# jiny2001/dcscn-super-resolution

Hardware: NVIDIA H100
Metric: output Mpixels/sec DCSCN L12 x2 (higher is better)
Workload: dtype f16x3 (fp16 hi/lo split operands, fp32 accumulate; fp32-equivalent)

## Files before the change

### dcscn-super-resolution_b200/csrc/conv_tc.cuh

```cuda
#pragma once
#include "common.h"
#include "epilogue.cuh"
#include "ptx.cuh"

namespace dcscn {

constexpr int kConsumerWGs = 2;
constexpr int kTcThreads = (1 + kConsumerWGs) * 128;
constexpr int kRegsIssue = 40, kRegsEpilogue = 232;
constexpr int kMaxASlots = 4;
constexpr int kMaxWSlots = 12;
constexpr int kTcBarrierBytes = 2 * (kMaxASlots + kMaxWSlots) * 8;
constexpr int kMaxTileN = 112;
constexpr int kRdotSmemBytes = 9 * 128 * 4;
constexpr int kColSplit = 2;
constexpr int kXchgStride = 36;
constexpr int kXchgBytes = kConsumerWGs * 64 * kXchgStride * 4;
constexpr int kTcKC = 64;

struct TcSmem {
  static constexpr int kRowBytes = kTcKC * 2;
  static constexpr int kSbo = 8 * kRowBytes;
  static constexpr uint64_t kLayout = 1ull;
};

__device__ __forceinline__ uint64_t make_smem_desc(uint32_t saddr) {
  return (uint64_t)((saddr & 0x3FFFFu) >> 4) | ((uint64_t)1 << 16) | ((uint64_t)(TcSmem::kSbo >> 4) << 32) |
         (TcSmem::kLayout << 62);
}

__host__ __device__ inline uint32_t tc_a_plane_bytes(int TW, int TH, int ksz) {
  return ((uint32_t)TW * (uint32_t)(TH + ksz - 1) * (uint32_t)kTcKC * 2u + 1023u) & ~1023u;
}
__host__ __device__ inline uint32_t tc_w_tile_bytes(int nplanes, int n_pad) {
  return (uint32_t)nplanes * (uint32_t)n_pad * (uint32_t)kTcKC * 2u;
}

template <int N, int NPLANES, int KS>
__device__ __forceinline__ void tile_products(float (&corr)[N / 2], float (&dom)[N / 2], uint64_t a_hi, uint64_t a_lo,
                                              uint64_t b_hi, uint64_t b_lo, uint32_t acc_on) {
  ptx::wgmma_fence();
#pragma unroll
  for (int ks = 0; ks < KS; ++ks) {
    const uint64_t kadd = (uint64_t)ks * 2u;
    const uint32_t on = ks == 0 ? acc_on : 1u;
    if (NPLANES == 2) {
      ptx::wgmma_f16<N, 0, 0>(corr, a_lo + kadd, b_hi + kadd, on);
      ptx::wgmma_f16<N, 0, 0>(corr, a_hi + kadd, b_lo + kadd, 1u);
    }
    ptx::wgmma_f16<N, 0, 0>(dom, a_hi + kadd, b_hi + kadd, on);
  }
  ptx::wgmma_commit();
}

template <int NPLANES, int N>
__global__ void __launch_bounds__(kTcThreads, 1)
conv_tc_kernel(const __grid_constant__ CUtensorMap tm_hi, const __grid_constant__ CUtensorMap tm_lo,
               const ConvTCParams p, const int a_slots, const int w_slots) {
  static_assert(N % 16 == 0 && N >= 16 && N <= kMaxTileN, "column tile width");
  extern __shared__ __align__(1024) uint8_t smem_raw[];
  uint8_t* smem = reinterpret_cast<uint8_t*>((reinterpret_cast<uintptr_t>(smem_raw) + 1023) & ~uintptr_t(1023));
  const ConvGeom& g = p.g;
  const int ksz = p.ksz;
  const uint32_t A_PLANE = tc_a_plane_bytes(g.TW, g.TH, ksz);
  const uint32_t A_SLOT = NPLANES * A_PLANE;
  const uint32_t A_TX = (uint32_t)NPLANES * (uint32_t)g.TW * (uint32_t)(g.TH + ksz - 1) * kTcKC * 2u;
  constexpr uint32_t B_BYTES = N * kTcKC * 2;
  constexpr uint32_t W_TILE = NPLANES * B_BYTES;
  uint8_t* a_ring = smem;
  uint8_t* w_ring = smem + (size_t)a_slots * A_SLOT;
  uint64_t* a_full = reinterpret_cast<uint64_t*>(w_ring + (size_t)w_slots * W_TILE);
  uint64_t* a_empty = a_full + kMaxASlots;
  uint64_t* w_full = a_empty + kMaxASlots;
  uint64_t* w_empty = w_full + kMaxWSlots;
  float* s_rdot = reinterpret_cast<float*>(w_empty + kMaxWSlots);
  float* s_xchg = s_rdot + kRdotSmemBytes / 4;

  const int wg = threadIdx.x >> 7;
  const int lane = threadIdx.x & 31;

  if (threadIdx.x == 0) {
    for (int s = 0; s < a_slots; ++s) {
      ptx::mbar_init(&a_full[s], 1);
      ptx::mbar_init(&a_empty[s], kConsumerWGs);
    }
    for (int s = 0; s < w_slots; ++s) {
      ptx::mbar_init(&w_full[s], 1);
      ptx::mbar_init(&w_empty[s], kConsumerWGs);
    }
    ptx::fence_barrier_init();
    ptx::fence_proxy_async();
  }
  if (p.epi.mode == EPI_D2S_RDOT)
    for (int i = threadIdx.x; i < p.epi.rdot_taps * p.epi.d2s_cout; i += blockDim.x) s_rdot[i] = p.epi.rdot_w[i];
  __syncthreads();

  const int tiles_per_img = g.tiles_x * g.tiles_y;
  const int num_items = g.n_img * tiles_per_img * p.n_tiles;
  const int half = ksz >> 1;
  const int chunks = p.chunks;

  if (wg == 0) {
    ptx::setmaxnreg_dec<kRegsIssue>();
    if (threadIdx.x == 0) {
      ptx::prefetch_tensormap(&tm_hi);
      if (NPLANES == 2) ptx::prefetch_tensormap(&tm_lo);
      int as = 0, ws = 0;
      uint32_t a_ph = 0, w_ph = 0;
      for (int item = blockIdx.x; item < num_items; item += gridDim.x) {
        const int n_tile = item % p.n_tiles;
        const int tile = item / p.n_tiles;
        const int img = tile / tiles_per_img;
        const int t2 = tile - img * tiles_per_img;
        const int ty = t2 / g.tiles_x, tx = t2 - ty * g.tiles_x;
        const int x0 = tx * g.TW - half, y0 = ty * g.TH - half;
        const uint8_t* wsrc = reinterpret_cast<const uint8_t*>(p.wpack) + (size_t)n_tile * ksz * ksz * chunks * W_TILE;
        for (int ch = 0; ch < chunks; ++ch) {
          for (int dx = 0; dx < ksz; ++dx) {
            ptx::mbar_wait(&a_empty[as], a_ph ^ 1);
            uint8_t* ad = a_ring + (size_t)as * A_SLOT;
            ptx::mbar_arrive_expect_tx(&a_full[as], A_TX);
            ptx::tma_load_4d(ad, &tm_hi, &a_full[as], ch * kTcKC, x0 + dx, y0, img);
            if (NPLANES == 2) ptx::tma_load_4d(ad + A_PLANE, &tm_lo, &a_full[as], ch * kTcKC, x0 + dx, y0, img);
            if (++as == a_slots) { as = 0; a_ph ^= 1; }
            for (int dy = 0; dy < ksz; ++dy) {
              ptx::mbar_wait(&w_empty[ws], w_ph ^ 1);
              uint8_t* wd = w_ring + (size_t)ws * W_TILE;
              ptx::mbar_arrive_expect_tx(&w_full[ws], W_TILE);
              const uint8_t* wtile = wsrc + (size_t)((dy * ksz + dx) * chunks + ch) * W_TILE;
              ptx::bulk_load(wd, wtile, W_TILE, &w_full[ws]);
              if (++ws == w_slots) { ws = 0; w_ph ^= 1; }
            }
          }
        }
      }
    }
  } else {
    ptx::setmaxnreg_inc<kRegsEpilogue>();
    const int cw = wg - 1;
    const int t = threadIdx.x & 127;
    const int wq = t >> 5;
    constexpr int nch = N >> 4;
    constexpr int per = (nch + kColSplit - 1) / kColSplit;
    const int n_total = p.n_tiles * N;
    const bool strict = p.seg_chunks == 1;
    const uint32_t a_ring_u32 = ptx::smem_u32(a_ring);
    const uint32_t w_ring_u32 = ptx::smem_u32(w_ring);
    const uint32_t a_off = (uint32_t)(cw * 64 * TcSmem::kRowBytes);
    const uint32_t dy_step = (uint32_t)(g.TW * TcSmem::kRowBytes);
    const int row = cw * 64 + (t >> 1);
    const int grp = t & 1;
    const int py = row / g.TW, px = row - py * g.TW;
    const int first_chunk = grp * per;
    const int my_chunks = (nch - first_chunk) < per ? ((nch - first_chunk) > 0 ? nch - first_chunk : 0) : per;
    float* xchg = s_xchg + cw * 64 * kXchgStride;
    auto release_a = [&](int s) { ptx::mbar_arrive_if(&a_empty[s], t == 0); };
    auto release_w = [&](int s) { ptx::mbar_arrive_if(&w_empty[s], t == 0); };
    int as = 0, ws = 0;
    uint32_t a_ph = 0, w_ph = 0;
    for (int item = blockIdx.x; item < num_items; item += gridDim.x) {
      const int n_tile = item % p.n_tiles;
      const int tile = item / p.n_tiles;
      const int img = tile / tiles_per_img;
      const int t2 = tile - img * tiles_per_img;
      const int ty = t2 / g.tiles_x, tx = t2 - ty * g.tiles_x;
      const int y = ty * g.TH + py, x = tx * g.TW + px;
      const bool valid = (y < g.H) && (x < g.W);

      float sum[N / 2], corr[N / 2], dom[N / 2];
#pragma unroll
      for (int i = 0; i < N / 2; ++i) sum[i] = 0.f;
      auto promote = [&]() {
        ptx::reg_fence(corr);
        ptx::reg_fence(dom);
#pragma unroll
        for (int i = 0; i < N / 2; ++i) {
          if (NPLANES == 2) sum[i] += corr[i];
          sum[i] += dom[i];
        }
      };
      uint32_t acc_on = 0;
      int seg_left = p.seg_chunks;
      int pend_w = -1, pend_a = -1;
      for (int ch = 0; ch < chunks; ++ch) {
        int ksteps = p.cin_pad - ch * kTcKC;
        ksteps = (ksteps > kTcKC ? kTcKC : ksteps) >> 4;
        for (int dx = 0; dx < ksz; ++dx) {
          ptx::mbar_wait(&a_full[as], a_ph);
          const uint32_t a_addr = a_ring_u32 + (uint32_t)as * A_SLOT + a_off;
          for (int dy = 0; dy < ksz; ++dy) {
            ptx::mbar_wait(&w_full[ws], w_ph);
            const uint32_t w_addr = w_ring_u32 + (uint32_t)ws * W_TILE;
            const uint64_t a_hi = make_smem_desc(a_addr + (uint32_t)dy * dy_step);
            const uint64_t a_lo = make_smem_desc(a_addr + (uint32_t)dy * dy_step + A_PLANE);
            const uint64_t b_hi = make_smem_desc(w_addr);
            const uint64_t b_lo = make_smem_desc(w_addr + B_BYTES);
            const bool a_done = dy == ksz - 1;
            if (strict) {
#pragma unroll 1
              for (int ks = 0; ks < ksteps; ++ks) {
                const uint64_t kadd = (uint64_t)ks * 2u;
                tile_products<N, NPLANES, 1>(corr, dom, a_hi + kadd, a_lo + kadd, b_hi + kadd, b_lo + kadd, acc_on);
                ptx::wgmma_wait<0>();
                promote();
              }
              release_w(ws);
              if (a_done) release_a(as);
            } else {
              if (ksteps == 4)
                tile_products<N, NPLANES, 4>(corr, dom, a_hi, a_lo, b_hi, b_lo, acc_on);
              else if (ksteps == 1)
                tile_products<N, NPLANES, 1>(corr, dom, a_hi, a_lo, b_hi, b_lo, acc_on);
              else if (ksteps == 2)
                tile_products<N, NPLANES, 2>(corr, dom, a_hi, a_lo, b_hi, b_lo, acc_on);
              else
                tile_products<N, NPLANES, 3>(corr, dom, a_hi, a_lo, b_hi, b_lo, acc_on);
              acc_on = 1;
              const bool item_end = a_done && dx == ksz - 1 && ch == chunks - 1;
              if (--seg_left == 0 || item_end) {
                ptx::wgmma_wait<0>();
                promote();
                acc_on = 0;
                seg_left = p.seg_chunks;
                if (pend_w >= 0) release_w(pend_w);
                if (pend_a >= 0) release_a(pend_a);
                release_w(ws);
                if (a_done) release_a(as);
                pend_w = pend_a = -1;
              } else {
                ptx::wgmma_wait<1>();
                if (pend_w >= 0) release_w(pend_w);
                if (pend_a >= 0) release_a(pend_a);
                pend_w = ws;
                pend_a = a_done ? as : -1;
              }
            }
            if (++ws == w_slots) { ws = 0; w_ph ^= 1; }
          }
          if (++as == a_slots) { as = 0; a_ph ^= 1; }
        }
      }
      ptx::wgmma_wait<0>();

      float v9[9];
#pragma unroll
      for (int i = 0; i < 9; ++i) v9[i] = 0.f;
      const int r0 = wq * 16 + (lane >> 2), cq = 2 * (lane & 3);
#pragma unroll
      for (int k = 0; k < per; ++k) {
        ptx::named_bar_sync(1 + cw, 128);
#pragma unroll
        for (int c = 0; c < nch; ++c) {
          if (c == k || c == per + k) {
            float* dst = xchg + (c == k ? 0 : 16);
#pragma unroll
            for (int h = 0; h < 2; ++h) {
              const int j = 2 * c + h;
              dst[r0 * kXchgStride + 8 * h + cq] = sum[4 * j];
              dst[r0 * kXchgStride + 8 * h + cq + 1] = sum[4 * j + 1];
              dst[(r0 + 8) * kXchgStride + 8 * h + cq] = sum[4 * j + 2];
              dst[(r0 + 8) * kXchgStride + 8 * h + cq + 1] = sum[4 * j + 3];
            }
          }
        }
        ptx::named_bar_sync(1 + cw, 128);
        if (k < my_chunks) {
          float v[16];
          const float4* srcp = reinterpret_cast<const float4*>(xchg + (t >> 1) * kXchgStride + grp * 16);
#pragma unroll
          for (int q = 0; q < 4; ++q) {
            const float4 f = srcp[q];
            v[4 * q] = f.x; v[4 * q + 1] = f.y; v[4 * q + 2] = f.z; v[4 * q + 3] = f.w;
          }
          const int cg = n_tile * N + (first_chunk + k) * 16;
          if (p.epi.mode == EPI_D2S_RDOT) {
            if (cg < p.epi.n_valid) {
              const int ij = cg / p.epi.d2s_cout, cc = cg - ij * p.epi.d2s_cout;
              rdot_accumulate16(p.epi, s_rdot, cg, cc, v, v9);
              const bool last = p.epi.rdot_parts > 1 ? k + 1 == my_chunks : cc + 16 == p.epi.d2s_cout;
              if (last && valid) rdot_flush(p.epi, g, img, y, x, ij, p.epi.rdot_parts > 1 ? cc / (per * 16) : 0, v9);
            }
          } else if (valid) {
            if (p.epi.mode == EPI_D2S_TAPS) taps_store16(p.epi, g, img, y, x, cg, v);
            else epilogue_store16(p.epi, g, n_total, img, y, x, cg, v);
          }
        }
      }
    }
  }

  __syncthreads();
}

}
```

### dcscn-super-resolution_b200/csrc/engine.cu

```cuda
#include <cuda.h>
#include <cudaTypedefs.h>
#include <cuda_fp16.h>
#include <cuda_runtime.h>

#include <algorithm>
#include <cmath>
#include <cstdarg>
#include <cstdio>
#include <cstring>
#include <map>
#include <memory>
#include <string>
#include <type_traits>
#include <utility>
#include <vector>

#include "../../include/dcscn_b200.h"
#include "common.h"
#include "conv_aux.cuh"
#include "conv_tc.cuh"
#include "conv_ds_tile.cuh"
#include "train.cuh"
#include "wgrad_tc.cuh"
#include "train_ds.cuh"
// ... 636 lines not shown
      if (rdot_fusable(np, fuse_unit)) {
        t.n_pad = np;
        t.n_tiles = (cout_cols + np - 1) / np;
        break;
      }
    }
  }
  t.n_valid = cout_cols;
  t.w_host.assign((size_t)ksz * ksz * cin * cout_cols, 0.f);
  t.bias_host.assign((size_t)t.n_tiles * t.n_pad, 0.f);
  t.alpha_host.assign((size_t)t.n_tiles * t.n_pad, 1.f);
  return t;
}

static int finalize_params_ds(dcscn_handle* h) {
  h->ds_ab = dcscn_handle::DsDev();
  h->ds.clear();
  h->ds.resize(h->layers.size());
  const int T = h->ds_total, L = h->cfg.layers;
  std::vector<float> ab_pw, ab_bias, ab_alpha;
  const int na = h->cfg.nin_filters, nb = h->cfg.nin_filters2;
  ab_pw.assign((size_t)T * (na + nb), 0.f);
  ab_bias.assign(na + nb, 0.f);
  ab_alpha.assign(na + nb, 1.f);
  const bool slopes = h->cfg.activator <= DCSCN_ACTIVATOR_LEAKY_RELU;
  for (size_t i = 0; i < h->layers.size(); ++i) {
    const LayerDef& l = h->layers[i];
    const std::vector<float>& dwv = P(h, l.scope + "/depthwise_W");
    const std::vector<float>& pwv = P(h, l.scope + "/pointwise_W");
    if (l.scope == "A1" || l.scope == "B1") {
      const int col0 = l.scope == "A1" ? 0 : na;
      int ci = 0;
      for (int li = 0; li < L; ++li)
        for (int k = 0; k < h->filters[li]; ++k, ++ci) {
          const int pos = h->ds_off[li] + k;
          for (int co = 0; co < l.cout; ++co)
            if (l.k == 1) ab_pw[(size_t)pos * (na + nb) + col0 + co] = dwv[ci] * pwv[(size_t)ci * l.cout + co];
        }
      const auto& B = P(h, l.scope + "/conv_B");
      for (int co = 0; co < l.cout; ++co) ab_bias[col0 + co] = B[co];
      layer_slopes(h, l, ab_alpha.data() + col0);
      continue;
    }
    if (h->ds[i].dw.upload(dwv) || h->ds[i].pw.upload(pwv)) return 1;
    if (l.bias && h->ds[i].bias.upload(P(h, l.scope + "/conv_B"))) return 1;
    if (l.act) {
      std::vector<float> a(l.cout);
      layer_slopes(h, l, a.data());
      if (slopes && h->ds[i].alpha.upload(a)) return 1;
    }
  }
  if (h->ds_ab.pw.upload(ab_pw) || h->ds_ab.bias.upload(ab_bias)) return 1;
  if (slopes && h->ds_ab.alpha.upload(ab_alpha)) return 1;
  h->params_dirty = false;
  return 0;
}

static int build_bwd_layers(dcscn_handle* h);
static int sync_host_params(dcscn_handle* h);

static void first_layer_vectors(const dcscn_handle* h, std::vector<float>& w, std::vector<float>& b, std::vector<float>& a) {
  const LayerDef* l = find_layer(h, "CNN1");
  const int taps = l->k * l->k, np = h->feat_w[0];
  w.assign((size_t)taps * np, 0.f);
  b.assign(np, 0.f);
  a.assign(np, 1.f);
  std::vector<float> tmp;
  const std::vector<float>& W = layer_filter(h, *l, tmp);
  for (int tp = 0; tp < taps; ++tp)
    for (int co = 0; co < l->cout; ++co) w[(size_t)tp * np + co] = W[(size_t)tp * l->cout + co];
  const auto& B = P(h, "CNN1/conv_B");
  for (int co = 0; co < l->cout; ++co) b[co] = B[co];
  layer_slopes(h, *l, a.data());
}

static int construct_tc_layers(dcscn_handle* h) {
  const dcscn_config& c = h->cfg;
  const int L = c.layers;
  for (int i = 1; i < L; ++i) {
    const std::string scope = "CNN" + std::to_string(i + 1);
    const LayerDef* l = find_layer(h, scope);
    TcLayer t = make_tc(scope, tc_ksz(h, *l), l->cin, l->cout, h->feat_w[i - 1]);
    for (int ci = 0; ci < l->cin; ++ci) t.in_map.push_back(ci);
    fuse_columns(h, t, scope, 0, 0);
    h->tcl.push_back(std::move(t));
  }
  {
    const LayerDef* a1 = find_layer(h, "A1");
    const LayerDef* b1 = find_layer(h, "B1");
    TcLayer t = make_tc("A1+B1", 1, a1->cin, h->a1_w + b1->cout, h->feat_pitch);
    for (int li = 0; li < L; ++li)
      for (int ci = 0; ci < h->filters[li]; ++ci) t.in_map.push_back(h->feat_off[li] + ci);
    fuse_columns(h, t, "A1", 0, 0);
    fuse_columns(h, t, "B1", h->a1_w, 0);
    h->tcl.push_back(std::move(t));
  }
  {
    const LayerDef* l = find_layer(h, "B2");
    TcLayer t = make_tc("B2", tc_ksz(h, *l), l->cin, l->cout, h->b1_w);
    for (int ci = 0; ci < l->cin; ++ci) t.in_map.push_back(ci);
    fuse_columns(h, t, "B2", 0, 0);
    h->tcl.push_back(std::move(t));
  }
  {
    const std::string scope = up_scope(h);
    const LayerDef* l = find_layer(h, scope);
    const int fuse_unit = find_layer(h, "R-CNN1")->k == 3 ? h->ps_out : 0;
    TcLayer t = make_tc(tconv(h) ? "Up-TCNN" : "Up-PS", tc_ksz(h, *l), l->cin, l->cout, h->nin_pitch,
                        two_stage_up(h) ? 0 : fuse_unit);
    for (int ci = 0; ci < c.nin_filters2; ++ci) t.in_map.push_back(ci);
    for (int ci = 0; ci < c.nin_filters; ++ci) t.in_map.push_back(h->b1_w + ci);
    fuse_columns(h, t, scope, 0, 0);
    h->tcl.push_back(std::move(t));
    if (two_stage_up(h)) {
      const LayerDef* l2 = find_layer(h, "Up-PS2/Up-PS2_CNN");
      TcLayer t2 = make_tc("Up-PS2", tc_ksz(h, *l2), l2->cin, l2->cout, h->mid_pitch, fuse_unit);
      for (int ci = 0; ci < l2->cin; ++ci) t2.in_map.push_back(ci);
      fuse_columns(h, t2, "Up-PS2/Up-PS2_CNN", 0, 0);
      h->tcl.push_back(std::move(t2));
    }
  }
  if (h->train_enabled && !uses_ds_tile(h) && build_bwd_layers(h)) return 1;
  return 0;
}

static int rdot_parts(int n_pad, int cout) {
  const int nch = n_pad >> 4, per16 = ((nch + kColSplit - 1) / kColSplit) * 16;
  if (cout <= 0 || per16 % cout == 0) return 1;
  return (cout % per16 == 0) ? cout / per16 : 1;
}

static bool last_fuses(const dcscn_handle* h, int n_pad) {
  const int cout = h->ps_out, nch = n_pad >> 4, per = (nch + kColSplit - 1) / kColSplit;
  return find_layer(h, "R-CNN1")->k == 3 && cout % 16 == 0 && cout <= 128 && nch % kColSplit == 0 &&
         ((per * 16) % cout == 0 || (rdot_parts(n_pad, cout) > 1 && n_pad % (per * 16) == 0));
}

static double fold_dot(const float* a, const float* w, int C) {
  double s = 0.0;
  for (int c = 0; c < C; ++c) s += (double)a[c] * (double)w[c];
  return s;
}

static TcLayer fold_shape(const TcLayer& up, int C) {
  TcLayer f;
  f.name = up.name;
  f.ksz = up.ksz;
  f.cin = up.cin;
  f.cin_pad = up.cin_pad;
  f.in_map = up.in_map;
  f.cout = f.n_valid = up.cout / C * 9;
  f.n_pad = up.n_pad;
  f.n_tiles = (f.cout + f.n_pad - 1) / f.n_pad;
  f.w_host.assign((size_t)f.ksz * f.ksz * f.cin * f.cout, 0.f);
  f.bias_host.assign((size_t)f.n_tiles * f.n_pad, 0.f);
  f.alpha_host.assign((size_t)f.n_tiles * f.n_pad, 1.f);
  f.dw_ksz = up.dw_ksz;
  f.dw_host = up.dw_host;
  return f;
}

static void build_fold(dcscn_handle* h) {
  h->fold = TcLayer();
  const TcLayer& up = h->tcl.back();
  if (planes(h) != 2 || !last_fuses(h, up.n_pad)) return;
  std::vector<float> tmp;
  const std::vector<float>& wr = layer_filter(h, *find_layer(h, "R-CNN1"), tmp);
  const int C = h->ps_out, sub = up.cout / C;
  TcLayer f = fold_shape(up, C);
  const size_t rows = (size_t)up.ksz * up.ksz * up.cin;
  for (size_t r = 0; r < rows; ++r)
    for (int ij = 0; ij < sub; ++ij)
      for (int t = 0; t < 9; ++t)
        f.w_host[r * f.cout + ij * 9 + t] = (float)fold_dot(&up.w_host[r * up.cout + (size_t)ij * C], &wr[(size_t)t * C], C);
  for (int ij = 0; ij < sub; ++ij)
    for (int t = 0; t < 9; ++t) f.bias_host[ij * 9 + t] = (float)fold_dot(&up.bias_host[(size_t)ij * C], &wr[(size_t)t * C], C);
  h->fold = std::move(f);
}

static void adopt_arrays(TcLayer& t, TcLayer& old) {
  t.d_wpack = std::move(old.d_wpack); t.d_bias = std::move(old.d_bias); t.d_alpha = std::move(old.d_alpha);
  t.d_wref = std::move(old.d_wref); t.d_in_map = std::move(old.d_in_map); t.d_img_map = std::move(old.d_img_map);
  t.d_dw = std::move(old.d_dw);
}

static int finalize_params(dcscn_handle* h) {
  const dcscn_config& c = h->cfg;
  if (sync_host_params(h)) return 1;
  if (uses_ds_tile(h)) return finalize_params_ds(h);
  std::vector<TcLayer> old_tcl = std::move(h->tcl);
  std::vector<TcLayer> old_bwd = std::move(h->bwd);
  TcLayer old_fold = std::move(h->fold);
  h->tcl.clear();
  h->bwd.clear();
  h->refresh_ready = false;
  bool moved = false;
  {
    std::vector<float> w, b, a;
    first_layer_vectors(h, w, b, a);
    if (h->d_first_w.upload(w, &moved) || h->d_first_bias.upload(b, &moved) || h->d_first_alpha.upload(a, &moved)) return 1;
  }
  if (construct_tc_layers(h)) return 1;
  auto repack = [&](std::vector<TcLayer>& cur, std::vector<TcLayer>& old) {
    for (size_t i = 0; i < cur.size(); ++i) {
      TcLayer& t = cur[i];
      if (i < old.size()) adopt_arrays(t, old[i]);
      if (pack_tc_layer(h, t, &moved)) return 1;
    }
    return 0;
  };
  if (repack(h->tcl, old_tcl) || repack(h->bwd, old_bwd)) return 1;
  build_fold(h);
  if (h->fold.cout > 0) {
    adopt_arrays(h->fold, old_fold);
    if (pack_tc_layer(h, h->fold, &moved)) return 1;
  }
  {
    std::vector<float> tmp;
    if (h->d_last_w.upload(layer_filter(h, *find_layer(h, "R-CNN1"), tmp), &moved)) return 1;
  }
  if (moved) {
    h->plans.clear();
    h->last_plan = nullptr;
  }
  h->graph_epoch++;
  h->params_dirty = false;
  return 0;
}

struct WorkspaceShape {
  size_t feat, b1, nin, mid;
  size_t u;
  size_t hr, vbuf;
  int planes;
  size_t bytes_per_px(bool ds) const {
    return ds ? 4 * (feat + b1 + nin + mid + hr) : 2 * (size_t)planes * (feat + b1 + nin + mid + u) + 4 * (hr + vbuf);
  }
};

static WorkspaceShape workspace_shape(const dcscn_handle* h) {
  const dcscn_config& c = h->cfg;
  const size_t s2 = (size_t)c.scale * c.scale;
  WorkspaceShape w;
  w.u = 0;
  if (uses_ds_tile(h)) {
    const int cps = c.nin_filters + c.nin_filters2;
    w.feat = h->ds_total;
    w.b1 = c.nin_filters2;
    w.nin = cps;
    w.mid = c.scale == 4 ? 4 * (size_t)cps : 0;
    w.hr = s2 * h->ps_out;
    w.vbuf = 0;
    w.planes = 1;
    return w;
  }
  w.feat = h->feat_pitch;
  w.b1 = h->b1_w;
  w.nin = h->nin_pitch;
  w.mid = two_stage_up(h) ? 4 * (size_t)h->mid_pitch : 0;
  w.hr = s2 * h->ps_out;
  w.vbuf = s2 * 9 * (size_t)rdot_parts(h->tcl.empty() ? 16 : h->tcl.back().n_pad, h->ps_out);
  w.planes = planes(h);
  if (h->ds_wide) {
    for (const LayerDef& l : h->layers) {
      if (!ds_split(h, l)) continue;
      const std::string& sc = l.scope;
      const size_t per_px = sc == "B2" ? w.b1 : sc == "Up-PS/Up-PS_CNN" ? w.nin : sc == "Up-PS2/Up-PS2_CNN" ? w.mid
                                                                          : (size_t)pad16(l.cin);
      w.u = std::max(w.u, per_px);
    }
  }
  return w;
}

static int ensure_workspace(dcscn_handle* h, size_t lr_px) {
  if (lr_px <= h->cap_px) return 0;
  const dcscn_config& c = h->cfg;
  const WorkspaceShape ws = workspace_shape(h);
  if (uses_ds_tile(h)) {
    if (h->ds_feat.alloc(lr_px * ws.feat, true)) return 1;
    if (h->ds_b1.alloc(lr_px * ws.b1) || h->ds_nin.alloc(lr_px * ws.nin)) return 1;
    if (c.scale == 4 && h->ds_mid.alloc(lr_px * ws.mid)) return 1;
    if (h->ds_hr.alloc(lr_px * ws.hr)) return 1;
    h->cap_px = lr_px;
    return 0;
  }
  h->plans.clear();
  h->last_plan = nullptr;
  const bool two = ws.planes == 2;
  if (h->feat.alloc(lr_px * ws.feat, two) || h->b1.alloc(lr_px * ws.b1, two) || h->nin.alloc(lr_px * ws.nin, two) ||
      h->mid.alloc(lr_px * ws.mid, two) || h->u.alloc(lr_px * ws.u, two))
    return 1;
  if (h->hr.alloc(lr_px * ws.hr, true) || h->vbuf.alloc(lr_px * ws.vbuf, true)) return 1;
  h->cap_px = lr_px;
  return 0;
}

static int64_t workspace_bytes(const dcscn_handle* h) {
  auto bytes = [](const auto&... a) { return (int64_t)(0 + ... + (a.size() * sizeof(*a.get()))); };
  return h->feat.bytes() + h->b1.bytes() + h->nin.bytes() + h->mid.bytes() + h->u.bytes() +
         bytes(h->hr, h->vbuf, h->ds_feat, h->ds_b1, h->ds_nin, h->ds_mid, h->ds_hr, h->tile_x, h->tile_x2, h->tile_y);
}

constexpr size_t kTcRingBudget = 227 * 1024 - 1024 - kTcBarrierBytes - kRdotSmemBytes - kXchgBytes;

static bool tc_patch_fits(int nplanes, int n_pad, int ksz, int TH, int TW) {
  if (ksz == 1) return true;
  if (TW % 8 != 0) return false;
  return 2 * (size_t)nplanes * tc_a_plane_bytes(TW, TH, ksz) + 2 * (size_t)tc_w_tile_bytes(nplanes, n_pad) <=
         kTcRingBudget;
}

static bool choose_patch(int H, int W, int nplanes, int n_pad, int ksz, int* TH, int* TW) {
  static const int cand[][2] = {{8, 16}, {4, 32}, {16, 8}, {2, 64}, {32, 4}, {1, 128}, {64, 2}, {128, 1}};
  long long best = -1;
  for (auto& c : cand) {
    const int th = c[0], tw = c[1];
    if (!tc_patch_fits(nplanes, n_pad, ksz, th, tw)) continue;
    long long area = (long long)((H + th - 1) / th) * th * ((W + tw - 1) / tw) * tw;
    if (best < 0 || area < best) {
      best = area;
      *TH = th;
      *TW = tw;
    }
  }
  return best >= 0;
}

static int encode_map(dcscn_handle* h, CUtensorMap* tm, const __half* base, int cin_pad, int pitch, int n, int H,
                      int W, int TH, int TW) {
  cuuint64_t dims[4] = {(cuuint64_t)cin_pad, (cuuint64_t)W, (cuuint64_t)H, (cuuint64_t)n};
  cuuint64_t strides[3] = {(cuuint64_t)pitch * 2, (cuuint64_t)W * pitch * 2, (cuuint64_t)H * W * pitch * 2};
  cuuint32_t box[4] = {(cuuint32_t)kTcKC, (cuuint32_t)TW, (cuuint32_t)TH, 1};
  cuuint32_t estr[4] = {1, 1, 1, 1};
  CUresult r = h->encode(tm, CU_TENSOR_MAP_DATA_TYPE_FLOAT16, 4, (void*)base, dims, strides, box, estr,
                         CU_TENSOR_MAP_INTERLEAVE_NONE, CU_TENSOR_MAP_SWIZZLE_128B,
                         CU_TENSOR_MAP_L2_PROMOTION_L2_256B, CU_TENSOR_MAP_FLOAT_OOB_FILL_NONE);
  if (r != CUDA_SUCCESS)
    return fail("cuTensorMapEncodeTiled failed (%d) cin_pad=%d pitch=%d n=%d H=%d W=%d box=%dx%d", (int)r, cin_pad,
                pitch, n, H, W, TH, TW);
  return 0;
}

static int add_tc_launch(dcscn_handle* h, Plan* pl, const TcLayer& t, PlaneView src, int src_pitch, int n, int H, int W,
                         const EpiParams& epi) {
  TcLaunch L;
  memset(&L, 0, sizeof(L));
  int TH = 0, TW = 0;
  if (!choose_patch(H, W, planes(h), t.n_pad, t.ksz, &TH, &TW))
    return fail("layer %s: no pixel patch fits a %dx%d filter in shared memory", t.name.c_str(), t.ksz, t.ksz);
  if (t.ksz > 1 && TW % 8 != 0)
    return fail("internal: layer %s: patch width %d is not a whole number of swizzle atoms", t.name.c_str(), TW);
  ConvGeom g{n, H, W, (W + TW - 1) / TW, (H + TH - 1) / TH, TW, TH};
  const int box_rows = TH + t.ksz - 1;
  if (encode_map(h, &L.tm_hi, src.hi, t.cin_pad, src_pitch, n, H, W, box_rows, TW)) return 1;
  if (planes(h) == 2) {
    if (encode_map(h, &L.tm_lo, src.lo, t.cin_pad, src_pitch, n, H, W, box_rows, TW)) return 1;
  } else {
    L.tm_lo = L.tm_hi;
  }
  L.p.g = g;
  L.p.ksz = t.ksz;
  L.p.cin_pad = t.cin_pad;
  L.p.chunks = (t.cin_pad + kTcKC - 1) / kTcKC;
  L.p.n_tiles = t.n_tiles;
  L.p.n_pad = t.n_pad;
  L.p.seg_chunks = h->seg_chunks > 0 ? h->seg_chunks : (t.n_pad > 64 ? 2 : 3);
  L.p.wpack = t.d_wpack.get();
  L.p.epi = epi;
  L.p.epi.bias = t.d_bias.get();
  L.p.epi.alpha = t.d_alpha.get();
  L.p.epi.out_scale = 1.0f / t.wscale;
  if (!h->tcl.empty() && &t >= h->tcl.data() && &t < h->tcl.data() + h->tcl.size()) {
    L.layer_index = (int)(&t - h->tcl.data());
    L.layer_bwd = false;
  } else if (!h->bwd.empty() && &t >= h->bwd.data() && &t < h->bwd.data() + h->bwd.size()) {
    L.layer_index = (int)(&t - h->bwd.data());
    L.layer_bwd = true;
  }
  L.p.epi.n_valid = t.n_valid;

  const size_t a_slot = (size_t)planes(h) * tc_a_plane_bytes(TW, TH, t.ksz);
  const size_t w_tile = tc_w_tile_bytes(planes(h), t.n_pad);
  const size_t budget = kTcRingBudget;
  int a_slots, w_slots;
  if (t.ksz == 1) {
    a_slots = w_slots = (int)std::min<size_t>(kMaxASlots, budget / (a_slot + w_tile));
  } else {
    a_slots = 3;
    if (budget < a_slots * a_slot + 4 * w_tile) a_slots = 2;
    w_slots = budget < a_slots * a_slot ? 0 : (int)std::min<size_t>(kMaxWSlots, (budget - a_slots * a_slot) / w_tile);
  }
  if (a_slots < 2 || w_slots < 2)
    return fail("layer %s: two %zu-byte activation slots and two %zu-byte weight tiles do not fit in shared memory",
                t.name.c_str(), a_slot, w_tile);
  L.a_slots = a_slots;
  L.w_slots = w_slots;
  L.smem = a_slots * a_slot + w_slots * w_tile + 1024 + kTcBarrierBytes + kRdotSmemBytes + kXchgBytes;
  const long long tiles = (long long)n * g.tiles_x * g.tiles_y;
  const long long items = tiles * t.n_tiles;
  L.grid = (int)std::min<long long>(items, h->sm_count);

  L.ref.g = g;
  L.ref.ksz = t.ksz;
  L.ref.cin = t.cin;
  L.ref.cout = t.cout;
  L.ref.src_hi = src.hi;
  L.ref.src_lo = src.lo;
  L.ref.src_pitch = src_pitch;
  L.ref.in_map = t.d_in_map.get();
  L.ref.w = t.d_wref.get();
  L.ref.n_total_pad = t.n_tiles * t.n_pad;
  L.ref.epi = L.p.epi;
  L.ref.epi.out_scale = 1.0f;
  pl->tc.push_back(L);
  return 0;
}

static int add_layer_launch(dcscn_handle* h, Plan* pl, const TcLayer& t, PlaneView src, int src_pitch, int n, int H, int W,
                            const EpiParams& epi) {
  DwParams d;
  memset(&d, 0, sizeof(d));
  if (t.dw_ksz) {
    const PlaneView u = h->u.at(0);
    d = DwParams{n, H, W, t.dw_ksz, t.cin_pad, src.hi, src.lo, src_pitch, t.d_dw.get(), u.hi, u.lo};
    src = u;
    src_pitch = t.cin_pad;
    pl->dw_count++;
  }
  pl->dw.push_back(d);
  return add_tc_launch(h, pl, t, src, src_pitch, n, H, W, epi);
}

static EpiParams epi_planes(PlaneView dst, int pitch, int cols) {
  EpiParams e;
  memset(&e, 0, sizeof(e));
  e.mode = EPI_PLANES;
  e.num_seg = 1;
  e.seg[0] = {0, cols, dst.hi, dst.lo, pitch};
  e.keep_prob = 1.0f;
  e.out_scale = 1.0f;
  return e;
}

static EpiParams epi_activated(const dcscn_handle* h, std::initializer_list<const ActView*> outs) {
  EpiParams e = epi_planes({}, 0, 0);
  e.num_seg = 0;
  for (const ActView* v : outs) {
    e.seg[e.num_seg++] = {v->drop_col0, v->drop_col0 + pad16(v->ch), v->planes.hi, v->planes.lo, v->pitch};
    e.drop_ntotal = v->drop_stride;
  }
  e.act = h->cfg.activator;
  return e;
}

static int add_activated_launch(dcscn_handle* h, Plan* pl, const TcLayer& t, const ActView& src, int n, int H, int W,
                                std::initializer_list<const ActView*> outs) {
  if (add_layer_launch(h, pl, t, src.planes, src.pitch, n, H, W, epi_activated(h, outs))) return 1;
  std::copy(outs.begin(), outs.end(), pl->tc.back().act);
  return 0;
}

static Plan* get_plan(dcscn_handle* h, int n, int H, int W) {
  for (auto& p : h->plans)
    if (p->n == n && p->h == H && p->w == W) return p.get();
  const dcscn_config& c = h->cfg;
  const int L = c.layers;
  std::unique_ptr<Plan> pl(new Plan());
  pl->n = n;
  pl->h = H;
  pl->w = W;
  pl->act.resize(h->layers.size());
  for (size_t li = 0; li < h->layers.size(); ++li)
    if (h->layers[li].act) act_view(h, h->layers[li].scope, &pl->act[li]);
  const ActView* a = pl->act.data();

  memset(&pl->first, 0, sizeof(pl->first));
  pl->first.g = ConvGeom{n, H, W, 1, 1, 1, 1};
  pl->first.ksz = find_layer(h, "CNN1")->k;
  pl->first.n_pad = h->feat_w[0];
  pl->first.w = h->d_first_w.get();
  pl->first.epi = epi_activated(h, {&a[0]});
  pl->first.epi.bias = h->d_first_bias.get();
  pl->first.epi.alpha = h->d_first_alpha.get();
  pl->first.epi.n_valid = h->filters[0];

  size_t ti = 0;
  for (int i = 1; i < L; ++i)
    if (add_activated_launch(h, pl.get(), h->tcl[ti++], a[i - 1], n, H, W, {&a[i]})) return nullptr;
  if (add_activated_launch(h, pl.get(), h->tcl[ti++], a[0], n, H, W, {&a[L], &a[L + 1]})) return nullptr;
  if (add_activated_launch(h, pl.get(), h->tcl[ti++], a[L + 1], n, H, W, {&a[L + 2]})) return nullptr;
  int HR_H = H, HR_W = W;
  {
    EpiParams e;
    memset(&e, 0, sizeof(e));
    e.keep_prob = 1.0f;
    if (two_stage_up(h)) {
      e.mode = EPI_D2S_PLANES;
      e.d2s_r = 2;
      e.d2s_cout = c.nin_filters + c.nin_filters2;
      e.num_seg = 1;
      e.seg[0] = {0, 0, h->mid.hi.get(), h->mid.lo.get(), h->mid_pitch};
    } else {
      e.mode = EPI_D2S_F32;
      e.d2s_r = c.scale;
      e.d2s_cout = h->ps_out;
      e.dst_f32 = h->hr.get();
      e.d2s_pitch = h->ps_out;
    }
    if (add_layer_launch(h, pl.get(), h->tcl[ti++], h->nin.at(0), h->nin_pitch, n, H, W, e)) return nullptr;
    HR_H = H * (two_stage_up(h) ? 2 : c.scale);
    HR_W = W * (two_stage_up(h) ? 2 : c.scale);
  }
  if (two_stage_up(h)) {
    EpiParams e;
    memset(&e, 0, sizeof(e));
    e.keep_prob = 1.0f;
    e.mode = EPI_D2S_F32;
    e.d2s_r = 2;
    e.d2s_cout = h->ps_out;
    e.dst_f32 = h->hr.get();
    e.d2s_pitch = h->ps_out;
    if (add_layer_launch(h, pl.get(), h->tcl[ti++], h->mid.at(0), h->mid_pitch, n, HR_H, HR_W, e)) return nullptr;
    HR_H *= 2;
    HR_W *= 2;
  }
  {
    TcLaunch& L = pl->tc.back();
    const int cout = h->ps_out, nch = L.p.n_pad >> 4, per = (nch + kColSplit - 1) / kColSplit;
    const int klast = find_layer(h, "R-CNN1")->k;
    const int parts = rdot_parts(L.p.n_pad, cout);
    pl->unfused = L;
    pl->fused_index = (int)pl->tc.size() - 1;
    pl->fused_last = last_fuses(h, L.p.n_pad);
    if (pl->fused_last && h->fold.cout > 0) {
      const TcLayer& f = h->fold;
      L.layer_index = -1;
      L.layer_fold = true;
      L.p.n_tiles = f.n_tiles;
      L.p.wpack = f.d_wpack.get();
      L.p.epi.bias = f.d_bias.get();
      L.p.epi.alpha = f.d_alpha.get();
      L.p.epi.out_scale = 1.0f / f.wscale;
      L.p.epi.n_valid = f.n_valid;
      L.p.epi.mode = EPI_D2S_TAPS;
      L.p.epi.rdot_out = h->vbuf.get();
      L.p.epi.rdot_taps = 9;
      L.p.epi.rdot_parts = 1;
      L.grid = (int)std::min<long long>((long long)n * L.p.g.tiles_x * L.p.g.tiles_y * f.n_tiles, h->sm_count);
    } else if (pl->fused_last) {
      L.p.epi.rdot_parts = ((per * 16) % cout == 0) ? 1 : parts;
      L.p.epi.mode = EPI_D2S_RDOT;
      L.p.epi.rdot_w = h->d_last_w.get();
      L.p.epi.rdot_out = h->vbuf.get();
      L.p.epi.rdot_taps = klast * klast;
    }
    const int gparts = pl->fused_last ? L.p.epi.rdot_parts : 1;
    memset(&pl->gather, 0, sizeof(pl->gather));
    pl->gather.parts = gparts;
    pl->gather.n_img = n;
    pl->gather.H = HR_H;
    pl->gather.W = HR_W;
    pl->gather.ksz = klast;
    pl->gather.v = h->vbuf.get();
  }
  memset(&pl->last, 0, sizeof(pl->last));
  pl->last.n_img = n;
  pl->last.H = HR_H;
  pl->last.W = HR_W;
  pl->last.ksz = find_layer(h, "R-CNN1")->k;
  pl->last.C = h->ps_out;
  pl->last.pitch = h->ps_out;
  pl->last.src = h->hr.get();
  pl->last.w = h->d_last_w.get();
  pl->last.bias = 0.f;
  if (h->plans.size() >= 64) h->plans.erase(h->plans.begin());
  h->plans.push_back(std::move(pl));
  return h->plans.back().get();
}

template <int NPL, int N>
static int launch_tc_inst(dcscn_handle* h, const TcLaunch& L, cudaStream_t st) {
  static bool attr_set_dev[64] = {};
  bool& attr_set = attr_set_dev[h->cfg.device_id & 63];
  if (!attr_set) {
    CUDA_TRY(cudaFuncSetAttribute(conv_tc_kernel<NPL, N>, cudaFuncAttributeMaxDynamicSharedMemorySize, 227 * 1024));
    attr_set = true;
  }
  conv_tc_kernel<NPL, N><<<L.grid, kTcThreads, L.smem, st>>>(L.tm_hi, L.tm_lo, L.p, L.a_slots, L.w_slots);
  CUDA_TRY(cudaGetLastError());
  return 0;
}

template <int NPL>
static int launch_tc_width(dcscn_handle* h, const TcLaunch& L, cudaStream_t st) {
  switch (L.p.n_pad) {
    case 16: return launch_tc_inst<NPL, 16>(h, L, st);
    case 32: return launch_tc_inst<NPL, 32>(h, L, st);
    case 48: return launch_tc_inst<NPL, 48>(h, L, st);
    case 64: return launch_tc_inst<NPL, 64>(h, L, st);
    case 80: return launch_tc_inst<NPL, 80>(h, L, st);
    case 96: return launch_tc_inst<NPL, 96>(h, L, st);
    case 112: return launch_tc_inst<NPL, 112>(h, L, st);
  }
  return fail("internal: column tile width %d is not a multiple of 16 in [16, %d]", L.p.n_pad, kMaxTileN);
}

static int launch_tc(dcscn_handle* h, const TcLaunch& Lc, cudaStream_t st) {
  h->launches++;
  TcLaunch& L = const_cast<TcLaunch&>(Lc);
  if (L.layer_fold) {
    L.p.epi.out_scale = 1.0f / h->fold.wscale;
  } else if (L.layer_index >= 0) {
    const std::vector<TcLayer>& ls = L.layer_bwd ? h->bwd : h->tcl;
    if (L.layer_index < (int)ls.size()) L.p.epi.out_scale = 1.0f / ls[L.layer_index].wscale;
  }
  if (h->conv_impl == 1) {
    const long long total = (long long)L.ref.g.n_img * L.ref.g.H * L.ref.g.W * (L.ref.n_total_pad >> 4);
    const int grid = (int)std::min<long long>((total + 127) / 128, (long long)h->sm_count * 16);
    conv_ref_kernel<<<grid, 128, 0, st>>>(L.ref);
    CUDA_TRY(cudaGetLastError());
    return 0;
  }
  const int npl = planes(h);
  if (L.p.wpack == nullptr) return fail("internal: weight image was not packed for this layer");
  return npl == 2 ? launch_tc_width<2>(h, L, st) : launch_tc_width<1>(h, L, st);
}

static int mark(dcscn_handle* h, cudaStream_t st) {
  if (!h->timing) return 0;
  if (h->ev_used >= (int)h->ev.size()) {
    cudaEvent_t e;
    CUDA_TRY(cudaEventCreate(&e));
    h->ev.emplace_back(e);
  }
  CUDA_TRY(cudaEventRecord(h->ev[h->ev_used++].get(), st));
  return 0;
}

template <int KSZ>
static int launch_ds_tile_k(dcscn_handle* h, const DsTileParams& p, unsigned grid, size_t smem, cudaStream_t st) {
  const int cols = p.cout < 32 ? ((p.cout + 3) & ~3) : 32;
  static size_t attr_dev[64][2] = {};
  size_t& cur = attr_dev[h->cfg.device_id & 63][KSZ == 3 ? 1 : 0];
  if (cur == 0) cur = 48 * 1024;
  if (smem > cur) {
    const int b = (int)smem;
    CUDA_TRY(cudaFuncSetAttribute(ds_tile_kernel<KSZ, 1>, cudaFuncAttributeMaxDynamicSharedMemorySize, b));
    CUDA_TRY(cudaFuncSetAttribute(ds_tile_kernel<KSZ, 2>, cudaFuncAttributeMaxDynamicSharedMemorySize, b));
    CUDA_TRY(cudaFuncSetAttribute(ds_tile_kernel<KSZ, 4>, cudaFuncAttributeMaxDynamicSharedMemorySize, b));
    CUDA_TRY(cudaFuncSetAttribute(ds_tile_kernel<KSZ, 6>, cudaFuncAttributeMaxDynamicSharedMemorySize, b));
    CUDA_TRY(cudaFuncSetAttribute(ds_tile_kernel<KSZ, 8>, cudaFuncAttributeMaxDynamicSharedMemorySize, b));
    cur = smem;
  }
  if (cols <= 4) ds_tile_kernel<KSZ, 1><<<grid, kDtThreads, smem, st>>>(p);
  else if (cols <= 8) ds_tile_kernel<KSZ, 2><<<grid, kDtThreads, smem, st>>>(p);
  else if (cols <= 16) ds_tile_kernel<KSZ, 4><<<grid, kDtThreads, smem, st>>>(p);
  else if (cols <= 24) ds_tile_kernel<KSZ, 6><<<grid, kDtThreads, smem, st>>>(p);
  else ds_tile_kernel<KSZ, 8><<<grid, kDtThreads, smem, st>>>(p);
  CUDA_TRY(cudaGetLastError());
  return 0;
}

static int launch_ds_tile(dcscn_handle* h, DsTileParams p, int ksz, cudaStream_t st) {
  if (ksz != 1 && ksz != 3) return fail("depthwise-separable layer: kernel size %d is not supported (1 or 3)", ksz);
  if (p.cout > 32 && p.cin > kDtCC) return fail("depthwise-separable layer %d -> %d: more than 32 output columns need <= 32 input channels", p.cin, p.cout);
  const size_t smem = ds_tile_launch_smem(ksz, p.cin, p.cout);
  if (smem > 200 * 1024) return fail("depthwise-separable layer %d -> %d exceeds the kernel's shared memory", p.cin, p.cout);
  unsigned grid;
  if (ksz == 3) {
    p.tiles_x = (p.W + kDtT - 1) / kDtT;
    p.tiles_y = (p.H + kDtT - 1) / kDtT;
    grid = (unsigned)((long long)p.n_img * p.tiles_x * p.tiles_y);
  } else {
    grid = (unsigned)(((long long)p.n_img * p.H * p.W + kDtThreads - 1) / kDtThreads);
  }
  const int rc = ksz == 3 ? launch_ds_tile_k<3>(h, p, grid, smem, st) : launch_ds_tile_k<1>(h, p, grid, smem, st);
  if (rc) return rc;
  h->launches++;
  return mark(h, st);
}

static DsTileParams ds_tile_params(const LayerDef& l, const dcscn_handle::DsDev& d, const float* src, int src_pitch, float* dst,
                                   int dst_pitch, int dst_off, int n, int H, int W) {
  DsTileParams p;
  memset(&p, 0, sizeof(p));
  p.n_img = n; p.H = H; p.W = W; p.cin = l.cin; p.cout = l.cout;
  p.src = src; p.src_pitch = src_pitch; p.dw = d.dw.get(); p.pw = d.pw.get(); p.bias = d.bias.get(); p.alpha = d.alpha.get();
  p.dst = dst; p.dst_pitch = dst_pitch; p.dst_off = dst_off;
  return p;
}

static int ds_activate(dcscn_handle* h, float* buf, long long npx, int pitch, int off, int C, cudaStream_t st) {
  if (h->cfg.activator < DCSCN_ACTIVATOR_SIGMOID) return 0;
  const long long total = npx * C;
  ds_act_kernel<<<(int)std::min<long long>((total + 255) / 256, (long long)h->sm_count * 16), 256, 0, st>>>(buf, npx, pitch, off, C,
                                                                                                          h->cfg.activator);
  CUDA_TRY(cudaGetLastError());
  h->launches++;
  return 0;
}

static int forward_ds_tile(dcscn_handle* h, const float* x, const float* x2, float* y, int n, int H, int W, cudaStream_t st) {
  const dcscn_config& c = h->cfg;
  const int L = c.layers, T = h->ds_total, na = c.nin_filters, nb = c.nin_filters2, cps = na + nb;
  if (!h->tiling) {
    h->ev_used = 0;
    if (mark(h, st)) return 1;
  }
  size_t li = 0;
  for (int i = 0; i < L; ++i, ++li) {
    const float* src = i == 0 ? x : h->ds_feat.get() + h->ds_off[i - 1];
    DsTileParams p = ds_tile_params(h->layers[li], h->ds[li], src, i == 0 ? c.channels : T, h->ds_feat.get(), T, h->ds_off[i], n, H, W);
    if (launch_ds_tile(h, p, h->layers[li].k, st)) return 1;
    if (ds_activate(h, h->ds_feat.get(), (long long)n * H * W, T, h->ds_off[i], h->filters[i], st)) return 1;
  }
  {
    if (h->layers[li].k != 1 || h->layers[li + 1].k != 1) return fail("depthwise-separable A1 / B1 must be 1x1");
    LayerDef ab = h->layers[li];
    ab.k = 1; ab.cin = T; ab.cout = cps;
    DsTileParams p = ds_tile_params(ab, h->ds_ab, h->ds_feat.get(), T, h->ds_nin.get(), cps, nb, n, H, W);
    p.dw = nullptr;
    p.split = na;
    p.dst2 = h->ds_b1.get(); p.dst2_pitch = nb; p.dst2_off = 0;
    if (cps > 32) return fail("depthwise-separable graph: nin_filters + nin_filters2 = %d > 32 is not supported by the fused A1|B1 kernel", cps);
    if (launch_ds_tile(h, p, 1, st)) return 1;
    if (ds_activate(h, h->ds_nin.get(), (long long)n * H * W, cps, nb, na, st) || ds_activate(h, h->ds_b1.get(), (long long)n * H * W, nb, 0, nb, st))
      return 1;
    li += 2;
  }
  {
    DsTileParams p = ds_tile_params(h->layers[li], h->ds[li], h->ds_b1.get(), nb, h->ds_nin.get(), cps, 0, n, H, W);
    if (launch_ds_tile(h, p, h->layers[li].k, st)) return 1;
    if (ds_activate(h, h->ds_nin.get(), (long long)n * H * W, cps, 0, nb, st)) return 1;
    ++li;
  }
  int HH = H, WW = W;
  if (c.scale == 4) {
    DsTileParams p = ds_tile_params(h->layers[li], h->ds[li], h->ds_nin.get(), cps, h->ds_mid.get(), cps, 0, n, H, W);
    p.d2s_r = 2; p.d2s_cout = cps;
    if (launch_ds_tile(h, p, h->layers[li].k, st)) return 1;
    ++li;
    HH = 2 * H; WW = 2 * W;
    DsTileParams q = ds_tile_params(h->layers[li], h->ds[li], h->ds_mid.get(), cps, h->ds_hr.get(), h->ps_out, 0, n, HH, WW);
    q.d2s_r = 2; q.d2s_cout = h->ps_out;
    if (launch_ds_tile(h, q, h->layers[li].k, st)) return 1;
    ++li;
    HH *= 2; WW *= 2;
  } else {
    DsTileParams p = ds_tile_params(h->layers[li], h->ds[li], h->ds_nin.get(), cps, h->ds_hr.get(), h->ps_out, 0, n, H, W);
    p.d2s_r = c.scale; p.d2s_cout = h->ps_out;
    if (launch_ds_tile(h, p, h->layers[li].k, st)) return 1;
    ++li;
    HH = c.scale * H; WW = c.scale * W;
  }
  if (h->wait_x2) {
    CUDA_TRY(cudaStreamWaitEvent(st, h->x2_ready.get(), 0));
    h->wait_x2 = false;
  }
  const LayerDef& lr = h->layers[li];
  const dcscn_handle::DsDev& d = h->ds[li];
  if (lr.cin == 1 && lr.cout == 1) {
    if (lr.k != 1 && lr.k != 3) return fail("depthwise-separable R-CNN1: kernel size %d is not supported (1 or 3)", lr.k);
    const long long total = (long long)n * HH * WW;
    const bool vec4 = lr.k == 3 && (WW & 3) == 0 && total < (1ll << 32) &&
                      ((reinterpret_cast<uintptr_t>(y) | reinterpret_cast<uintptr_t>(x2)) & 15) == 0 &&
                      (!h->tiling || h->tile_vec4);
    const int grid = (int)std::min<long long>(((vec4 ? total / 4 : total) + 255) / 256, (long long)h->sm_count * 16);
    if (vec4) ds_single4_kernel<<<grid, 256, 0, st>>>(h->ds_hr.get(), x2, y, n, HH, WW, d.dw.get(), d.pw.get(), d.bias.get(), d.alpha.get());
    else if (lr.k == 3) ds_single_kernel<3><<<grid, 256, 0, st>>>(h->ds_hr.get(), x2, y, n, HH, WW, d.dw.get(), d.pw.get(), d.bias.get(), d.alpha.get());
    else ds_single_kernel<1><<<grid, 256, 0, st>>>(h->ds_hr.get(), x2, y, n, HH, WW, d.dw.get(), d.pw.get(), d.bias.get(), d.alpha.get());
    CUDA_TRY(cudaGetLastError());
    h->launches++;
    return mark(h, st);
  }
  DsTileParams p = ds_tile_params(lr, d, h->ds_hr.get(), h->ps_out, y, 1, 0, n, HH, WW);
  p.add = x2;
  return launch_ds_tile(h, p, lr.k, st);
}

static int launch_depthwise(dcscn_handle* h, const DwParams& p, cudaStream_t st) {
  const long long total = (long long)p.n_img * p.H * p.W * (p.cpad >> 3);
  const int grid = (int)std::min<long long>((total + 255) / 256, (long long)h->sm_count * 16);
  if (p.ksz == 3) depthwise_planes_kernel<3><<<grid, 256, 0, st>>>(p);
  else if (p.ksz == 5) depthwise_planes_kernel<5><<<grid, 256, 0, st>>>(p);
  else return fail("depthwise step: kernel size %d is not supported (3 or 5)", p.ksz);
  CUDA_TRY(cudaGetLastError());
  h->launches++;
  return mark(h, st);
}

static int launch_first(dcscn_handle* h, const ConvFirstParams& p, cudaStream_t st) {
  if (p.ksz > 5) return fail("cnn_size %d is not supported by the first-layer kernel", p.ksz);
  const long long total = (long long)p.g.n_img * p.g.H * p.g.W;
  if (p.ksz == 3 && p.n_pad <= 256) {
    const int grid = (int)std::min<long long>((total + 7) / 8, (long long)h->sm_count * 8);
    if (p.epi.seg[0].dst_zneg != nullptr) conv_first3x3_kernel<true><<<grid, 256, 0, st>>>(p);
    else conv_first3x3_kernel<false><<<grid, 256, 0, st>>>(p);
  } else {
    const int grid = (int)std::min<long long>((total + 255) / 256, (long long)h->sm_count * 8);
    conv_first_kernel<<<grid, 256, (size_t)p.ksz * p.ksz * p.n_pad * sizeof(float), st>>>(p);
  }
  CUDA_TRY(cudaGetLastError());
  h->launches++;
  return 0;
}

static int issue_front(dcscn_handle* h, Plan* pl, const float* x, bool fused, cudaStream_t st) {
  ConvFirstParams first = pl->first;
  first.x = x;
  if (launch_first(h, first, st) || mark(h, st)) return 1;
  for (size_t i = 0; i < pl->tc.size(); ++i) {
    if (pl->dw[i].ksz && launch_depthwise(h, pl->dw[i], st)) return 1;
    const TcLaunch& L = ((int)i == pl->fused_index && !fused) ? pl->unfused : pl->tc[i];
    if (launch_tc(h, L, st)) return 1;
    if (mark(h, st)) return 1;
  }
  return 0;
}

static int forward_impl(dcscn_handle* h, const float* x, const float* x2, float* y, int n, int H, int W,
                        cudaStream_t st) {
  if (n <= 0 || H <= 0 || W <= 0) return fail("forward: bad shape n=%d h=%d w=%d", n, H, W);
  CUDA_TRY(cudaSetDevice(h->cfg.device_id));
  if (h->params_dirty && finalize_params(h)) return 1;
  if (ensure_workspace(h, (size_t)n * H * W)) return 1;
  if (!h->tiling) h->tiled_last = false;
  if (uses_ds_tile(h)) {
    h->ds_n = n; h->ds_h = H; h->ds_w = W;
    return forward_ds_tile(h, x, x2, y, n, H, W, st);
  }
  Plan* pl = get_plan(h, n, H, W);
  if (!pl) return 1;
  h->last_plan = pl;
  if (!h->tiling) {
    h->ev_used = 0;
    if (mark(h, st)) return 1;
  }
  const bool fused = pl->fused_last && h->fuse_last && h->conv_impl == 0;

  const bool graphable = h->use_graph && !h->timing && h->conv_impl == 0;
  if (graphable && pl->gexec && pl->g_x == x && pl->g_epoch == h->graph_epoch && pl->g_fused == fused) {
    CUDA_TRY(cudaGraphLaunch(pl->gexec, st));
    h->launches += pl->g_launches;
    h->graph_replays++;
  } else if (graphable && pl->eager_runs >= 1 && pl->last_x == x) {
    if (!h->cap_stream) {
      cudaStream_t s;
      CUDA_TRY(cudaStreamCreateWithFlags(&s, cudaStreamNonBlocking));
      h->cap_stream.reset(s);
    }
    if (pl->gexec) { cudaGraphExecDestroy(pl->gexec); pl->gexec = nullptr; }
    const int64_t before = h->launches;
    CUDA_TRY(cudaStreamBeginCapture(h->cap_stream.get(), cudaStreamCaptureModeThreadLocal));
    const int rc = issue_front(h, pl, x, fused, h->cap_stream.get());
    cudaGraph_t g = nullptr;
    const cudaError_t ce = cudaStreamEndCapture(h->cap_stream.get(), &g);
    h->launches = before;
    if (rc) { if (g) cudaGraphDestroy(g); return 1; }
    if (ce != cudaSuccess || g == nullptr) return fail("forward: stream capture failed: %s", cudaGetErrorString(ce));
    const cudaError_t ie = cudaGraphInstantiate(&pl->gexec, g, 0);
    cudaGraphDestroy(g);
    if (ie != cudaSuccess) { pl->gexec = nullptr; return fail("forward: cudaGraphInstantiate failed: %s", cudaGetErrorString(ie)); }
    pl->g_x = x; pl->g_epoch = h->graph_epoch; pl->g_fused = fused;
    pl->g_launches = 1 + pl->dw_count + (int)pl->tc.size();
    CUDA_TRY(cudaGraphLaunch(pl->gexec, st));
    h->launches += pl->g_launches;
    h->graph_replays++;
  } else {
    if (issue_front(h, pl, x, fused, st)) return 1;
    pl->eager_runs++;
  }
  pl->last_x = x;
  pl->ran_fused = fused;
  if (h->wait_x2) {
    CUDA_TRY(cudaStreamWaitEvent(st, h->x2_ready.get(), 0));
    h->wait_x2 = false;
  }
  if (fused) {
    ConvGatherParams p = pl->gather;
    p.x2 = x2;
    p.y = y;
    const size_t total = (size_t)p.n_img * p.H * p.W;
    const bool vec4 = p.ksz == 3 && (p.W & 3) == 0 && ((reinterpret_cast<uintptr_t>(x2) | reinterpret_cast<uintptr_t>(y)) & 15) == 0 &&
                      (!h->tiling || h->tile_vec4);
    if (vec4) {
      const int grid = (int)std::min<size_t>((total / 4 + 255) / 256, (size_t)h->sm_count * 16);
      conv_last_gather4_kernel<<<grid, 256, 0, st>>>(p);
    } else {
      const int grid = (int)std::min<size_t>((total + 255) / 256, (size_t)h->sm_count * 16);
      conv_last_gather_kernel<<<grid, 256, 0, st>>>(p);
    }
// ... 1065 lines not shown
```

Before: 169.2.

## Use three consumer warpgroups for narrow column tiles to enlarge pixel tiles

For column tiles of width 64 or less, the tensor-core conv kernel now launches three consumer warpgroups instead of two, so each CTA covers 192 output pixels per tile. Register budgets per warpgroup are lowered to fit the extra warps, and the patch-shape search gains new 192-pixel candidates. Candidates are now filtered to match the per-width tile pixel count. The aim is more wgmma work per loaded weight tile and better amortisation of the producer, at the cost of lower register headroom, larger activation slots and possibly fewer ring slots.

```diff
diff --git a/dcscn-super-resolution_b200/csrc/conv_tc.cuh b/dcscn-super-resolution_b200/csrc/conv_tc.cuh
--- a/dcscn-super-resolution_b200/csrc/conv_tc.cuh
+++ b/dcscn-super-resolution_b200/csrc/conv_tc.cuh
@@ -5,17 +5,24 @@
 
 namespace dcscn {
 
-constexpr int kConsumerWGs = 2;
-constexpr int kTcThreads = (1 + kConsumerWGs) * 128;
 constexpr int kRegsIssue = 40, kRegsEpilogue = 232;
+constexpr int kRegsIssue3 = 32, kRegsEpilogue3 = 160;
 constexpr int kMaxASlots = 4;
 constexpr int kMaxWSlots = 12;
 constexpr int kTcBarrierBytes = 2 * (kMaxASlots + kMaxWSlots) * 8;
 constexpr int kMaxTileN = 112;
+constexpr int kMaxTileN3 = 64;
 constexpr int kRdotSmemBytes = 9 * 128 * 4;
 constexpr int kColSplit = 2;
 constexpr int kXchgStride = 36;
-constexpr int kXchgBytes = kConsumerWGs * 64 * kXchgStride * 4;
+
+__host__ __device__ constexpr int tc_consumer_wgs(int n) { return n <= kMaxTileN3 ? 3 : 2; }
+__host__ __device__ constexpr int tc_tile_pixels(int n) { return 64 * tc_consumer_wgs(n); }
+__host__ __device__ constexpr int tc_xchg_bytes(int n) { return tc_consumer_wgs(n) * 64 * kXchgStride * 4; }
+template <int N>
+constexpr int kWGs = tc_consumer_wgs(N);
+template <int N>
+constexpr int kTcThreads = (1 + kWGs<N>) * 128;
 constexpr int kTcKC = 64;
 
 struct TcSmem {
@@ -54,7 +61,7 @@
 }
 
 template <int NPLANES, int N>
-__global__ void __launch_bounds__(kTcThreads, 1)
+__global__ void __launch_bounds__(kTcThreads<N>, 1)
 conv_tc_kernel(const __grid_constant__ CUtensorMap tm_hi, const __grid_constant__ CUtensorMap tm_lo,
                const ConvTCParams p, const int a_slots, const int w_slots) {
   static_assert(N % 16 == 0 && N >= 16 && N <= kMaxTileN, "column tile width");
@@ -82,11 +89,11 @@
   if (threadIdx.x == 0) {
     for (int s = 0; s < a_slots; ++s) {
       ptx::mbar_init(&a_full[s], 1);
-      ptx::mbar_init(&a_empty[s], kConsumerWGs);
+      ptx::mbar_init(&a_empty[s], kWGs<N>);
     }
     for (int s = 0; s < w_slots; ++s) {
       ptx::mbar_init(&w_full[s], 1);
-      ptx::mbar_init(&w_empty[s], kConsumerWGs);
+      ptx::mbar_init(&w_empty[s], kWGs<N>);
     }
     ptx::fence_barrier_init();
     ptx::fence_proxy_async();
@@ -101,7 +108,7 @@
   const int chunks = p.chunks;
 
   if (wg == 0) {
-    ptx::setmaxnreg_dec<kRegsIssue>();
+    ptx::setmaxnreg_dec<kWGs<N> == 3 ? kRegsIssue3 : kRegsIssue>();
     if (threadIdx.x == 0) {
       ptx::prefetch_tensormap(&tm_hi);
       if (NPLANES == 2) ptx::prefetch_tensormap(&tm_lo);
@@ -136,7 +143,7 @@
       }
     }
   } else {
-    ptx::setmaxnreg_inc<kRegsEpilogue>();
+    ptx::setmaxnreg_inc<kWGs<N> == 3 ? kRegsEpilogue3 : kRegsEpilogue>();
     const int cw = wg - 1;
     const int t = threadIdx.x & 127;
     const int wq = t >> 5;
diff --git a/dcscn-super-resolution_b200/csrc/engine.cu b/dcscn-super-resolution_b200/csrc/engine.cu
--- a/dcscn-super-resolution_b200/csrc/engine.cu
+++ b/dcscn-super-resolution_b200/csrc/engine.cu
@@ -962,21 +962,26 @@
          bytes(h->hr, h->vbuf, h->ds_feat, h->ds_b1, h->ds_nin, h->ds_mid, h->ds_hr, h->tile_x, h->tile_x2, h->tile_y);
 }
 
-constexpr size_t kTcRingBudget = 227 * 1024 - 1024 - kTcBarrierBytes - kRdotSmemBytes - kXchgBytes;
+static size_t tc_ring_budget(int n_pad) {
+  return 227 * 1024 - 1024 - kTcBarrierBytes - kRdotSmemBytes - tc_xchg_bytes(n_pad);
+}
 
 static bool tc_patch_fits(int nplanes, int n_pad, int ksz, int TH, int TW) {
   if (ksz == 1) return true;
   if (TW % 8 != 0) return false;
   return 2 * (size_t)nplanes * tc_a_plane_bytes(TW, TH, ksz) + 2 * (size_t)tc_w_tile_bytes(nplanes, n_pad) <=
-         kTcRingBudget;
+         tc_ring_budget(n_pad);
 }
 
 static bool choose_patch(int H, int W, int nplanes, int n_pad, int ksz, int* TH, int* TW) {
-  static const int cand[][2] = {{8, 16}, {4, 32}, {16, 8}, {2, 64}, {32, 4}, {1, 128}, {64, 2}, {128, 1}};
+  static const int cand[][2] = {{8, 16}, {4, 32}, {16, 8}, {2, 64}, {32, 4}, {1, 128}, {64, 2}, {128, 1},
+                                {24, 8}, {12, 16}, {8, 24}, {6, 32}, {4, 48}, {3, 64}, {2, 96}, {1, 192},
+                                {48, 4}, {96, 2}, {192, 1}};
+  const int pixels = tc_tile_pixels(n_pad);
   long long best = -1;
   for (auto& c : cand) {
     const int th = c[0], tw = c[1];
-    if (!tc_patch_fits(nplanes, n_pad, ksz, th, tw)) continue;
+    if (th * tw != pixels || !tc_patch_fits(nplanes, n_pad, ksz, th, tw)) continue;
     long long area = (long long)((H + th - 1) / th) * th * ((W + tw - 1) / tw) * tw;
     if (best < 0 || area < best) {
       best = area;
@@ -1042,7 +1047,7 @@
 
   const size_t a_slot = (size_t)planes(h) * tc_a_plane_bytes(TW, TH, t.ksz);
   const size_t w_tile = tc_w_tile_bytes(planes(h), t.n_pad);
-  const size_t budget = kTcRingBudget;
+  const size_t budget = tc_ring_budget(t.n_pad);
   int a_slots, w_slots;
   if (t.ksz == 1) {
     a_slots = w_slots = (int)std::min<size_t>(kMaxASlots, budget / (a_slot + w_tile));
@@ -1056,7 +1061,7 @@
                 t.name.c_str(), a_slot, w_tile);
   L.a_slots = a_slots;
   L.w_slots = w_slots;
-  L.smem = a_slots * a_slot + w_slots * w_tile + 1024 + kTcBarrierBytes + kRdotSmemBytes + kXchgBytes;
+  L.smem = a_slots * a_slot + w_slots * w_tile + 1024 + kTcBarrierBytes + kRdotSmemBytes + tc_xchg_bytes(t.n_pad);
   const long long tiles = (long long)n * g.tiles_x * g.tiles_y;
   const long long items = tiles * t.n_tiles;
   L.grid = (int)std::min<long long>(items, h->sm_count);
@@ -1247,7 +1252,7 @@
     CUDA_TRY(cudaFuncSetAttribute(conv_tc_kernel<NPL, N>, cudaFuncAttributeMaxDynamicSharedMemorySize, 227 * 1024));
     attr_set = true;
   }
-  conv_tc_kernel<NPL, N><<<L.grid, kTcThreads, L.smem, st>>>(L.tm_hi, L.tm_lo, L.p, L.a_slots, L.w_slots);
+  conv_tc_kernel<NPL, N><<<L.grid, kTcThreads<N>, L.smem, st>>>(L.tm_hi, L.tm_lo, L.p, L.a_slots, L.w_slots);
   CUDA_TRY(cudaGetLastError());
   return 0;
 }
```

After: 170.8 (median of 6 runs). About the same (+0.9%).
